# adelacvg/detail_tts

Measured on AMD Instinct MI355X. Metric: generated audio seconds/sec (24 kHz), 10 s prompt, batch 8 per GPU, higher is better.
Workload: dtype f32; 1 GPU; configs[2]: 1xMI355X batch-8, 10 s prompts (T_ref=936), 234 codes -> 9.984 s audio per utterance; GPT KV-cache decode + 50-step CFG diffusion + flow-VAE/HiFiGAN vocoder, seed-0 random-init weights; batch_per_gpu=8, codes=234, diffusion_steps=50, parallelism=replica x1

## Files before the change

detail_tts_amd/csrc/attention.h:

```cpp
#pragma once
#include "common.h"

namespace dtts {

struct AttnParams {
    const float* qkv = nullptr;
    long long bs = 0;
    int cs = 0;
    int q_off = 0, k_off = 0, v_off = 0, head_stride = 0;
    float* out = nullptr;
    long long o_bs = 0;
    int o_cs = 0;
    const int* lens = nullptr;
    int T = 0, B = 0, H = 0, D = 0;
    float scale = 1.f;
    const float* bias_tab = nullptr;
    int causal = 0;
    const float* band = nullptr;
    int band_w = 0;
    float* ml_out = nullptr;
    int layout_pad = 0;
    void* out_x3 = nullptr;
    int x3_tp = 0;
    const void* planes = nullptr;
    int p1 = 0;
    int ksplit = 1;
    int ksplit_max = 0;
    float* kpart = nullptr;
    int* kcount = nullptr;
};

struct AttnPlanes {
    static constexpr int D = 48, KT = 64, TILE_BYTES = 2 * (6 * 64 + 8 * 48) * 16;
    __host__ __device__ static inline int tq(int T) { return (T + KT - 1) / KT * KT; }
    __host__ __device__ static inline int nt64(int T) { return (T + KT - 1) / KT; }
    __host__ __device__ static inline size_t q_bytes(int T) { return (size_t)2 * 6 * tq(T) * 16; }
    __host__ __device__ static inline size_t head_bytes(int T) { return q_bytes(T) + (size_t)nt64(T) * TILE_BYTES; }
    __host__ __device__ static inline size_t bytes(int B, int H, int T) { return (size_t)B * H * head_bytes(T); }
};

struct AttnX3Launch {
    int ksplit = 0, p1 = 0, workgroups = 0;
};
void launch_flash_attention(const AttnParams& p, hipStream_t stream, AttnX3Launch* chosen = nullptr);
// ... 13 lines not shown
```

detail_tts_amd/csrc/attention_x3b.hip:

```cpp
#include <atomic>
#include <type_traits>

#include "attention.h"
#include "conv_x3.h"
#include "split3.h"

namespace dtts {

namespace {
typedef float f16v __attribute__((ext_vector_type(16)));

constexpr int D = 48, KT = 64, QPW = 32, BIAS_CLIP = 64;
constexpr int KCH = 6 * KT;
constexpr int NPL = XS_PLANES;
constexpr int KBYTES = NPL * KCH * 16;
constexpr int VPLANE_G = 8 * D * 16;
constexpr int VHALF = 4 * D * 16;
constexpr int VSLOT = NPL * VHALF;
constexpr int EXT_HALF = 128, EXT_N = 2 * EXT_HALF + 1;
constexpr int ONES_BYTES = VHALF + 2 * D * 16 + 16;
constexpr int LDS_K = 0, LDS_V = 2 * KBYTES, LDS_ONES = LDS_V + 4 * VSLOT, LDS_EXT = LDS_ONES + 16, LDS_BYTES = LDS_ONES + ONES_BYTES;
static_assert(16 + EXT_N * 4 <= 2 * D * 16, "the bias table fits between the two ones chunks");
static_assert(3 * ((LDS_BYTES + 511) / 512 * 512) <= 160 * 1024, "three workgroups per CU");
constexpr float QK_SCALE = 16.f, P_SHIFT = 10.f, V_SCALE = 16.f, M_SLACK = 3.f;
// ... 213 lines not shown
    asm volatile("s_nop 7\n\ts_nop 7\n\ts_nop 7" : "+v"(a), "+v"(b));
}

template <int MINB, bool KSPLIT = false, bool ONEP = false>
__global__ __launch_bounds__(256, MINB) void flash_attn_x3b_kernel(const AttnParams p) {
    constexpr float LOG2E = 1.4426950408889634f;
    constexpr int NW = 4, QPB = NW * QPW;
    extern __shared__ __attribute__((aligned(16))) unsigned char smem[];
    float* ext_s = reinterpret_cast<float*>(smem + LDS_EXT);

    const int tid = threadIdx.x, lane = tid & 63, wave = __builtin_amdgcn_readfirstlane(tid >> 6);
    const int q = lane & 31, hh = lane >> 5;
    const int nqb = (p.T + QPB - 1) / QPB;
    const int S = KSPLIT ? p.ksplit : 1;
    const int Lall = xcd_remap(blockIdx.x, gridDim.x);
    const int Lid = KSPLIT ? Lall / S : Lall, zsp = KSPLIT ? Lall - Lid * S : 0;
    const int qb = Lid % nqb, hb = Lid / nqb;
    const int b = hb % p.B, h = hb / p.B;
    const int len = p.lens ? p.lens[b] : p.T;
    const int q0 = qb * QPB;
    if (q0 >= len) return;
    const int Tq = AttnPlanes::tq(p.T);
    const unsigned char* himg = static_cast<const unsigned char*>(p.planes) + ((size_t)b * p.H + h) * AttnPlanes::head_bytes(p.T);
    const unsigned char* kvimg = himg + AttnPlanes::q_bytes(p.T);
    for (int i = tid; i < EXT_N; i += NW * 64) {
        int o = i - EXT_HALF;
        o = o < -BIAS_CLIP ? -BIAS_CLIP : (o > BIAS_CLIP ? BIAS_CLIP : o);
        ext_s[i] = p.bias_tab[h * (2 * BIAS_CLIP + 1) + o + BIAS_CLIP] * LOG2E;
    }
    if (tid < 16) {
        const int c = tid >> 2;
        reinterpret_cast<unsigned*>(smem + LDS_ONES + (c >> 1) * VHALF + (c & 1) * (2 * D * 16))[tid & 3] = (c >> 1) ? 0u : 0x4C004C00u;
    }
// ... 207 lines not shown

void launch_flash_attention_x3b(const AttnParams& p, hipStream_t stream, AttnX3Launch* chosen) {
    DTTS_REQUIRE(p.D == 48 && p.bias_tab && !p.causal && !p.band && !p.ml_out && p.planes, "attention_x3b covers head dim 48 with the T5 bias on operand images");
    constexpr int NW = 4;
    const int base = cdiv(p.T, NW * QPW) * p.H * p.B;
    const int ks_env = attn_ksplit();
    static const int ks_maxb = env_int("DTTS_ATTN_KSPLIT_MAXB", 2);
    const int ks_cus = attn_ksplit_cus();
    int S = 1;
    if (p.B <= ks_maxb && ks_env > 1) {
        S = ks_env;
        while (S > 1 && ((long long)base * S > ks_cus || AttnPlanes::nt64(p.T) < 2 * S || (size_t)base * S > X3_MAX_SLABS || (size_t)base * NW > X3_SPLIT_COUNTERS)) --S;
    }
    if (p.ksplit_max > 0) S = std::min(S, p.ksplit_max);
    AttnParams q = p;
    if (S > 1) {
        q.ksplit = S;
        x3_split_workspace(stream, (size_t)base * S, &q.kpart, &q.kcount);
    }
    if (chosen) {
        chosen->ksplit = S;
        chosen->p1 = p.p1 ? 1 : 0;
        chosen->workgroups = base * S;
    }
    auto go = [&](auto kern) {
        lds_optin(reinterpret_cast<const void*>(kern), LDS_BYTES);
        hipLaunchKernelGGL(kern, dim3(base * S), dim3(NW * 64), LDS_BYTES, stream, q);
    };
    if (S > 1) {
        if (p.p1) go(flash_attn_x3b_kernel<2, true, true>);
// ... 10 lines not shown
```

detail_tts_amd/csrc/conv_gemm.h:

```cpp
#pragma once
#include "common.h"

namespace dtts {

struct ConvParams {
    const float* x = nullptr;
    long long x_bs = 0;
    int x_cs = 0;
    const int* len_in = nullptr;
    const int* x_bidx = nullptr;
    int Tin = 0;
    const float* pro_ab = nullptr;
    int pro_act = ACT_NONE;
    float pro_slope = 0.f;
    const float* w = nullptr;
    const float* bias = nullptr;
    int Cin = 0, CinP = 0, Cout = 0, CoutP = 0, KW = 1, stride = 1, dil = 1, pad = 0;
    const float* badd = nullptr;
    int badd_bs = 0;
    int gate = GATE_NONE;
    int epi_act = ACT_NONE;
    float epi_slope = 0.f;
    float out_scale = 1.f;
    const float* res = nullptr;
// ... 18 lines not shown
    int qkv_heads = 0, qkv_nt64 = 0, qkv_tq = 0;
    float qkv_qscale = 1.f;
    const int* cols = nullptr;
    int ncols = 0, cols_b0 = 0;
    void* next3 = nullptr;
    int next_c8 = 0, next_tp = 0, next_halo = 0, next_act = ACT_NONE;
    float next_slope = 0.f;
    int* next_sat = nullptr;
    int ksplit = 1;
    int ksplit_max = 0;
    int p1 = 0;
    int epi_vec = 0;
    float* kpart = nullptr;
    int* kcount = nullptr;
    int ablate = 0;
};

void launch_conv_gemm(const ConvParams& p, hipStream_t stream);
void set_conv_small_tiles(int n);

}
```

detail_tts_amd/csrc/conv_x3.hip:

```cpp
#include <algorithm>
#include <atomic>
#include <cstdio>
#include <mutex>
#include <type_traits>
#include <utility>
#include <vector>

#include "conv_x3.h"
#include <cstdlib>
#include "prof.h"
#include "split3.h"

namespace dtts {

typedef float f32x16 __attribute__((ext_vector_type(16)));

namespace {
constexpr int NPL = XS_PLANES, NK = 2 * NPL;
constexpr int BM = 128, BN = X3_BN;
constexpr int WTILE = NK * BM * 16;
constexpr int XMAIN = NK * BN * 16;
constexpr int XBUF = XMAIN + NK * 2 * 16;

__global__ __launch_bounds__(256) void split_weights_kernel(const float* __restrict__ wp, int C8, int CoutP, uint4* __restrict__ out) {
// ... 3 lines not shown
#pragma unroll
    for (int e = 0; e < 8; ++e) v[e] = wp[((long long)tap * C8 * 8 + c8 * 8 + e) * CoutP + m] * XS_SCALE_W;
    uint4 q0, q1;
    split8(v, q0, q1);
    uint4* o = out + ((long long)(tap * C8 + c8) * NPL) * CoutP + m;
    o[0] = q0;
    o[CoutP] = q1;
}

template <int ACT, bool AB>
__global__ __launch_bounds__(256) void split_planes_kernel(const float* __restrict__ x, long long x_bs, int x_cs,
                                                          const float* __restrict__ ab, const int* __restrict__ lens, int T, int C8,
                                                          int Tp, uint4* __restrict__ out) {
    const int tp = blockIdx.x * 256 + threadIdx.x, c8 = blockIdx.y, b = blockIdx.z;
    if (tp >= Tp) return;
    const int t = tp - X3_HALO, len = lens ? lens[b] : T;
    uint4 q0 = make_uint4(0, 0, 0, 0), q1 = q0;
    if (t >= 0 && t < len) {
        const float* xr = x + (long long)b * x_bs + (long long)(c8 * 8) * x_cs + t;
        float v[8];
#pragma unroll
        for (int e = 0; e < 8; ++e) v[e] = xr[(long long)e * x_cs];
        if (AB) {
            const float* abr = ab + ((long long)b * C8 + c8) * 16;
#pragma unroll
            for (int e = 0; e < 8; ++e) v[e] = abr[2 * e] * v[e] + abr[2 * e + 1];
        }
        if (ACT == ACT_SILU) {
#pragma unroll
            for (int e = 0; e < 8; ++e) v[e] = v[e] * __frcp_rn(1.f + __expf(-v[e]));
        }
#pragma unroll
        for (int e = 0; e < 8; ++e) v[e] *= XS_SCALE_X;
        split8(v, q0, q1);
    }
    uint4* o = out + ((long long)(b * C8 + c8) * NPL) * Tp + tp;
    o[0] = q0;
    o[Tp] = q1;
}

template <int ACT>
__global__ __launch_bounds__(1024) void gn_split_planes_kernel(const float* __restrict__ x, long long x_bs, int x_cs,
                                                              const int* __restrict__ lens, int T, int C, int groups,
                                                              const float* __restrict__ gamma, const float* __restrict__ beta, float eps,
                                                              const float* __restrict__ ada, int ada_stride, int ada_bs, int Tp,
                                                              uint4* __restrict__ out, const int* __restrict__ ada_idx, int x_bmod) {
    __shared__ float red[2][16];
    __shared__ float sa[64], sd[64];
    const int g = blockIdx.x, b = blockIdx.y, tid = threadIdx.x, lane = tid & 63, wave = tid >> 6, nthr = blockDim.x;
// ... 79 lines not shown
                v[e] *= XS_SCALE_X;
            }
            split8(v, q0, q1);
        }
        uint4* o = out + ((long long)(b * C8 + g * c8n + c8l) * NPL) * Tp + tp;
        o[0] = q0;
        o[Tp] = q1;
    }
}

template <int ACT, int NI>
__global__ __launch_bounds__(1024) void gn_split_planes_reg_kernel(const float* __restrict__ x, long long x_bs, int x_cs,
                                                                  const int* __restrict__ lens, int T, int C, int groups,
                                                                  const float* __restrict__ gamma, const float* __restrict__ beta, float eps,
                                                                  const float* __restrict__ ada, int ada_stride, int ada_bs, int Tp,
                                                                  uint4* __restrict__ out, const int* __restrict__ ada_idx, int x_bmod) {
    __shared__ float red[2][16];
    __shared__ float sa[64], sd[64];
    const int g = blockIdx.x, b = blockIdx.y, tid = threadIdx.x, lane = tid & 63, wave = tid >> 6;
    const int len = lens ? lens[b] : T;
    const int cpg = C / groups, c8n = cpg >> 3, C8 = C >> 3, nitems = c8n * Tp;
    const float* xg = x + (long long)(x_bmod ? b % x_bmod : b) * x_bs + (long long)(g * cpg) * x_cs;
    const float k = xg[0];
    float v[NI][8];
    float s1 = 0.f, s2 = 0.f;
#pragma unroll
    for (int q = 0; q < NI; ++q) {
        const int item = tid + q * 1024, c8l = item / Tp, t = item - c8l * Tp - X3_HALO;
        const bool ok = item < nitems && t >= 0 && t < len;
        const float* xr = xg + (long long)(ok ? c8l * 8 : 0) * x_cs + (ok ? t : 0);
#pragma unroll
        for (int e = 0; e < 8; ++e) v[q][e] = xr[(long long)e * x_cs];
        if (ok) {
            float d[8];
#pragma unroll
            for (int e = 0; e < 8; ++e) d[e] = v[q][e] - k;
            s1 += ((d[0] + d[1]) + (d[2] + d[3])) + ((d[4] + d[5]) + (d[6] + d[7]));
            s2 += ((d[0] * d[0] + d[1] * d[1]) + (d[2] * d[2] + d[3] * d[3])) + ((d[4] * d[4] + d[5] * d[5]) + (d[6] * d[6] + d[7] * d[7]));
        }
    }
#pragma unroll
    for (int o = 32; o > 0; o >>= 1) {
        s1 += __shfl_xor(s1, o);
        s2 += __shfl_xor(s2, o);
    }
    if (lane == 0) { red[0][wave] = s1; red[1][wave] = s2; }
    __syncthreads();
    float S1 = 0.f, S2 = 0.f;
// ... 9 lines not shown
        float d = beta[c] - mean * a;
        if (ada) {
            const float* ad = ada + (ada_idx ? (long long)ada_idx[b] : (long long)b * ada_bs);
            const float sc = 1.f + ad[(long long)c * ada_stride], sh = ad[(long long)(C + c) * ada_stride];
            a *= sc;
            d = d * sc + sh;
        }
        sa[tid] = a;
        sd[tid] = d;
    }
    __syncthreads();
#pragma unroll
    for (int q = 0; q < NI; ++q) {
        const int item = tid + q * 1024;
        if (item >= nitems) continue;
        const int c8l = item / Tp, tp = item - c8l * Tp, t = tp - X3_HALO;
        uint4 q0 = make_uint4(0, 0, 0, 0), q1 = q0;
        if (t >= 0 && t < len) {
            float w[8];
#pragma unroll
            for (int e = 0; e < 8; ++e) {
                w[e] = sa[c8l * 8 + e] * v[q][e] + sd[c8l * 8 + e];
                if (ACT == ACT_SILU) w[e] = w[e] * __frcp_rn(1.f + __expf(-w[e]));
                w[e] *= XS_SCALE_X;
            }
            split8(w, q0, q1);
        }
        uint4* o = out + ((long long)(b * C8 + g * c8n + c8l) * NPL) * Tp + tp;
        o[0] = q0;
        o[Tp] = q1;
    }
}

template <int EPI, bool KW3, int NSTG, bool P1 = false>
__global__ __launch_bounds__(256, NSTG == 2 ? 3 : 2) void conv_x3_kernel(ConvParams p) {
    constexpr int KW = KW3 ? 3 : 1, D = NSTG - 1;
    constexpr int CB = P1 ? 4 : 2;
    constexpr int NT = P1 ? 2 : 3;
    auto chunk_of = [](int kind) { return P1 ? kind * NPL : (kind & 1) * NPL + (kind >> 1); };
    constexpr int XOFF = NSTG * WTILE;
    extern __shared__ __attribute__((aligned(16))) unsigned char smem[];
    const int tid = threadIdx.x, lane = tid & 63, wave = __builtin_amdgcn_readfirstlane(tid >> 6), l31 = lane & 31, lhi = lane >> 5;
    const int mtiles = p.CoutP / BM, ntiles = (p.Nout + BN - 1) / BN;
    const int Ls = xcd_remap(blockIdx.x, gridDim.x);
    const int S = p.ksplit, L = Ls / S, z = Ls - L * S;
    int mt = L % mtiles;
    int b = (L / mtiles) / ntiles;
    int nti = (L / mtiles) - b * ntiles;
    int bn = L / mtiles;
    if (EPI == 2 && mtiles > 6 && mtiles % 6 == 0 && !(p.ablate & 1024)) {
        const int nbn = p.cols ? p.ncols : ntiles * p.B, per_blk = 5 * mtiles, blk = L / per_blk, r = L - blk * per_blk;
        const int bn0 = blk * 5, nb = min(5, nbn - bn0), per_grp = nb * 6, mg = r / per_grp, r2 = r - mg * per_grp, bnl = r2 / 6;
        mt = mg * 6 + (r2 - bnl * 6);
        bn = bn0 + bnl;
        b = bn / ntiles;
        nti = bn - b * ntiles;
    }
    if (p.cols) {
        const int pk = __builtin_amdgcn_readfirstlane(p.cols[bn]);
        b = (pk >> 8) - p.cols_b0;
        nti = pk & 255;
    }
    const int m0 = mt * BM, n0 = nti * BN;
    const int nvalid = p.len_out ? p.len_out[b] : p.Nout;
    if (n0 >= nvalid) return;
    const int C8 = p.Cin >> 3, call = p.Cin >> (P1 ? 5 : 4), Tp = p.x3_tp;
    const int cbeg = (int)((long long)call * z / S), c16n = (int)((long long)call * (z + 1) / S) - cbeg, nks = KW * c16n;
    const int bin = p.x_bidx ? p.x_bidx[b] : b;
    const unsigned lane16 = (unsigned)lane * 16u;
    const unsigned char* wb8 = static_cast<const unsigned char*>(p.w3) + ((long long)m0 + (long long)(CB * cbeg) * NPL * p.CoutP) * 16;
    const unsigned char* xb8 = static_cast<const unsigned char*>(p.x3) +
                               ((long long)bin * C8 * NPL * Tp + n0 + (X3_HALO - p.pad) + (long long)(CB * cbeg) * NPL * Tp) * 16;
    const long long wtapB = (long long)C8 * NPL * p.CoutP * 16;
    const long long wblkB = (long long)CB * NPL * p.CoutP * 16;
    const long long xblkB = (long long)CB * NPL * Tp * 16;
    auto dma = [&](const unsigned char* g, int lds_off) {
        __builtin_amdgcn_global_load_lds((const __attribute__((address_space(1))) void*)(g + lane16),
                                         (__attribute__((address_space(3))) void*)(smem + lds_off), 16, 0, 0);
    };
    const int wkind = wave;
    const unsigned char* wq = wb8 + (long long)chunk_of(wkind) * p.CoutP * 16;
    const int wlds = wkind * (BM * 16);
    const unsigned char* xq = xb8 + (long long)chunk_of(wkind) * Tp * 16;
    const int xlds = XOFF + wkind * (BN * 16);
    long long x3o[3];
    int x3l[3];
#pragma unroll
    for (int t = 0; t < 3; ++t) {
        const int j = t * 4 + wave, kind = j / 3, cb = j - kind * 3;
        x3o[t] = ((long long)chunk_of(kind) * Tp + cb * 64) * 16;
        x3l[t] = XOFF + kind * (BN * 16) + cb * 1024;
    }
    const long long halo_lane = (lane < 2 * NK) ? (((long long)chunk_of(lane >> 1) * Tp + BN + (lane & 1)) * 16 - (long long)lane16) : 0;
    const unsigned char* xblk = xb8;
    auto issue_w = [&](int i, int stage) { dma(wq + i * 1024, stage * WTILE + wlds + i * 1024); };
    auto issue_x1 = [&](int i, int stage) { dma(xq + i * 1024, stage * XBUF + xlds + i * 1024); };
    auto issue_x3 = [&](int t, int stage) { dma(xblk + x3o[t], stage * XBUF + x3l[t]); };
    auto issue_halo = [&](int stage) {
        if (lane < 2 * NK)
            __builtin_amdgcn_global_load_lds((const __attribute__((address_space(1))) void*)(xblk + halo_lane + lane16),
                                             (__attribute__((address_space(3))) void*)(smem + XOFF + stage * XBUF + XMAIN), 16, 0, 0);
    };
    int itap = 0;
    auto next_w = [&]() {
        if (!KW3) wq += wblkB;
        else if (itap < 2) { wq += wtapB; ++itap; }
        else { wq += wblkB - 2 * wtapB; itap = 0; }
    };

    const int wm0 = (wave >> 1) * 64, wn0 = (wave & 1) * 96;
    f32x16 acc[2][3];
#pragma unroll
    for (int i = 0; i < 2; ++i)
#pragma unroll
        for (int j = 0; j < 3; ++j)
#pragma unroll
            for (int r = 0; r < 16; ++r) acc[i][j][r] = 0.f;

#pragma unroll
    for (int q = 0; q < D; ++q) {
        if (q < nks) {
            issue_w(0, q);
            issue_w(1, q);
        }
        next_w();
        if (!KW3) {
            if (q < nks) {
#pragma unroll
                for (int i = 0; i < 3; ++i) issue_x1(i, q);
            }
            xq += xblkB;
        } else {
            if (q < c16n) {
#pragma unroll
                for (int t = 0; t < 3; ++t) issue_x3(t, q);
                issue_halo(q);
            }
            xblk += xblkB;
        }
    }
    float* bias_s = reinterpret_cast<float*>(smem + XOFF + NSTG * XBUF);
    if (tid < BM) bias_s[tid] = (p.bias && m0 + tid < p.Cout) ? p.bias[m0 + tid] : 0.f;

    int c16 = 0, tap = 0;
    int sw = 0, sx = 0;
    auto read_frags = [&](hf8 (&fa)[2][NPL], hf8 (&fb)[3][NPL], int stw, int stx, int tp) {
        const unsigned char* As = smem + stw * WTILE + lhi * (BM * 16);
        const unsigned char* Xb = smem + XOFF + stx * XBUF;
#pragma unroll
        for (int j = 0; j < 3; ++j) {
            const int nn = wn0 + j * 32 + l31 + tp;
            const unsigned char* xr = nn < BN ? Xb + lhi * (BN * 16) + nn * 16 : Xb + XMAIN + lhi * 32 + (nn - BN) * 16;
            const int xps = nn < BN ? 2 * BN * 16 : 64;
#pragma unroll
            for (int pl = 0; pl < NPL; ++pl) fb[j][pl] = *reinterpret_cast<const hf8*>(xr + pl * xps);
        }
#pragma unroll
// ... 74 lines not shown
#pragma unroll
        for (; slot < 5; ++slot) uslot(slot);
        if (!KW3) {
            wq += wblkB;
            xq += xblkB;
        } else {
            if ((TAPc + D) % KW < 2) wq += wtapB;
            else wq += wblkB - 2 * wtapB;
            if (TAPc == KW - 1) xblk += xblkB;
        }
    };
    auto uperiod = [&](auto... kc) { (ustep(kc), ...); };
    constexpr bool UNROLL = KW3 || EPI == 2;
    if (UNROLL && !(p.ablate & 512)) {
        const int nper = KW3 ? (c16n - D) / NSTG : (nks - D) / PERIOD;
        for (int q = 0; q < nper; ++q) {
            if constexpr (PERIOD == 2) uperiod(std::integral_constant<int, 0>{}, std::integral_constant<int, 1>{});
            else if constexpr (PERIOD == 3) uperiod(std::integral_constant<int, 0>{}, std::integral_constant<int, 1>{}, std::integral_constant<int, 2>{});
            else if constexpr (PERIOD == 4) uperiod(std::integral_constant<int, 0>{}, std::integral_constant<int, 1>{}, std::integral_constant<int, 2>{}, std::integral_constant<int, 3>{});
            else if constexpr (PERIOD == 6) uperiod(std::integral_constant<int, 0>{}, std::integral_constant<int, 1>{}, std::integral_constant<int, 2>{}, std::integral_constant<int, 3>{}, std::integral_constant<int, 4>{}, std::integral_constant<int, 5>{});
            else if constexpr (PERIOD == 9) uperiod(std::integral_constant<int, 0>{}, std::integral_constant<int, 1>{}, std::integral_constant<int, 2>{}, std::integral_constant<int, 3>{}, std::integral_constant<int, 4>{}, std::integral_constant<int, 5>{}, std::integral_constant<int, 6>{}, std::integral_constant<int, 7>{}, std::integral_constant<int, 8>{});
            else uperiod(std::integral_constant<int, 0>{}, std::integral_constant<int, 1>{}, std::integral_constant<int, 2>{}, std::integral_constant<int, 3>{}, std::integral_constant<int, 4>{}, std::integral_constant<int, 5>{}, std::integral_constant<int, 6>{}, std::integral_constant<int, 7>{}, std::integral_constant<int, 8>{}, std::integral_constant<int, 9>{}, std::integral_constant<int, 10>{}, std::integral_constant<int, 11>{});
        }
        ks = nper * PERIOD;
        c16 = ks / KW;
        itap = D % KW;
    }
    for (; ks < nks; ++ks) {
        if (NSTG == 2 || ks + D > nks || (KW3 && c16 + D >= c16n)) asm volatile("s_waitcnt vmcnt(0)" ::: "memory");
        else asm volatile("s_waitcnt vmcnt(%0)" ::"n"((NSTG - 2) * (KW3 ? 3 : 5)) : "memory");
        __builtin_amdgcn_s_barrier();
        read_frags(a, bb, sw, sx, tap);
        const int swi = sw + D >= NSTG ? sw + D - NSTG : sw + D, sxi = sx + D >= NSTG ? sx + D - NSTG : sx + D;
        const bool wlive = ks + D < nks, xlive = KW3 ? c16 + D < c16n : ks + D < nks;
        int slot = 0;
#pragma unroll
        for (int t = 0; t < NT; ++t)
#pragma unroll
            for (int i = 0; i < 2; ++i) {
#pragma unroll
                for (int j = 0; j < 3; ++j) acc[i][j] = __builtin_amdgcn_mfma_f32_32x32x16_f16(a[i][TA[t]], bb[j][TB[t]], acc[i][j], 0, 0, 0);
                if (slot < 5) issue_slot(slot, swi, sxi, wlive, xlive);
                ++slot;
            }
// ... 322 lines not shown
}

void launch_gn_split_planes(const float* x, long long x_bs, int x_cs, const int* lens, int T, int B, int C, int groups,
                            const float* gamma, const float* beta, float eps, const float* ada, int ada_stride, int ada_bs, int act,
                            void* out, hipStream_t s, const int* ada_idx, int x_bmod) {
    DTTS_REQUIRE(C % groups == 0 && (C / groups) % 8 == 0 && C / groups <= 64, "gn_split_planes: group size");
    DTTS_REQUIRE(act == ACT_NONE || act == ACT_SILU, "gn_split_planes: activation");
    const int Tp = x3_tp(T);
    uint4* o = static_cast<uint4*>(out);
    ProfScope ps("gn_split_planes_kernel", 0.0, (double)B * C * T * 8.0, s);
    static const int ns = env_int("DTTS_GN_SPLIT_NS", 1);
    static const int nt = env_int("DTTS_GN_SPLIT_NT", 1024);
    static const bool reg_ok = env_on("DTTS_GN_SPLIT_REG");
    constexpr int NI = 3;
    if (reg_ok && ns == 1 && (C / groups / 8) * Tp <= NI * 1024) {
        if (act == ACT_SILU)
            hipLaunchKernelGGL((gn_split_planes_reg_kernel<ACT_SILU, NI>), dim3(groups, B), dim3(1024), 0, s, x, x_bs, x_cs, lens, T, C, groups,
                               gamma, beta, eps, ada, ada_stride, ada_bs, Tp, o, ada_idx, x_bmod);
        else
            hipLaunchKernelGGL((gn_split_planes_reg_kernel<ACT_NONE, NI>), dim3(groups, B), dim3(1024), 0, s, x, x_bs, x_cs, lens, T, C, groups,
                               gamma, beta, eps, ada, ada_stride, ada_bs, Tp, o, ada_idx, x_bmod);
        DTTS_CHECK_HIP(hipGetLastError());
        return;
    }
    if (act == ACT_SILU)
        hipLaunchKernelGGL(gn_split_planes_kernel<ACT_SILU>, dim3(groups, B, ns), dim3(nt), 0, s, x, x_bs, x_cs, lens, T, C, groups, gamma,
                           beta, eps, ada, ada_stride, ada_bs, Tp, o, ada_idx, x_bmod);
    else
        hipLaunchKernelGGL(gn_split_planes_kernel<ACT_NONE>, dim3(groups, B, ns), dim3(nt), 0, s, x, x_bs, x_cs, lens, T, C, groups, gamma,
                           beta, eps, ada, ada_stride, ada_bs, Tp, o, ada_idx, x_bmod);
    DTTS_CHECK_HIP(hipGetLastError());
}

namespace {
struct KSplitWs {
    float* part;
// ... 85 lines not shown
    const long long ntile_pad = (long long)(p.CoutP / BM) * cdiv(p.Nout, BN) * p.B;
    static const int max_split_k1 = env_int("DTTS_CONV_KSPLIT_K1", 2);
    if (ntile_pad <= split_tiles) S = (int)std::min<long long>(std::min<long long>(p.KW == 3 ? max_split : std::min(max_split, max_split_k1), split_wgs / ntile_pad), (p.Cin >> 4) / 8);
    if (p.ksplit_max > 0) S = std::min(S, p.ksplit_max);
    if (S < 1) S = 1;
    p.ksplit = S;
    static const bool epi_vec_on = env_on("DTTS_X3_EPI_VEC");
    auto al16 = [](const void* q, long long bs, int cs) { return (reinterpret_cast<unsigned long long>(q) & 15ull) == 0 && (bs & 3) == 0 && (cs & 3) == 0; };
    p.epi_vec = (epi_vec_on && p.y && al16(p.y, p.y_bs, p.y_cs) && (!p.res || al16(p.res, p.res_bs, p.res_cs))) ? 1 : 0;
    if (S > 1) {
        const KSplitWs w = ksplit_workspace(s, (size_t)ntile * S);
        p.kpart = w.part;
        p.kcount = w.count;
    }
    const long long nwg = ntile * S;
    static const long long max4k3 = env_int("DTTS_CONV_STAGES4_MAXWG_K3", 128);
    const int nstg = force_stg ? force_stg : (nwg <= (p.KW == 3 ? max4k3 : max4) ? 4 : (nwg <= max3 ? 3 : 2));
    const size_t lds = (size_t)nstg * (WTILE + XBUF) + BM * sizeof(float) + 16;
    const int l4 = 4 * (WTILE + XBUF) + BM * (int)sizeof(float) + 16;
    const dim3 grid((unsigned)nwg);
    const double cols = (double)p.B * p.Nout;
    const double flops = 2.0 * p.Cout * p.Cin * p.KW * cols;
    const double bytes = 4.0 * cols * p.Cin + 4.0 * cols * p.Cout * (p.res ? 2.0 : 1.0) + 4.0 * (double)p.Cout * p.Cin * p.KW;
    {
        static const bool by_shape = []() { const char* v = env_str("DTTS_PROF_SHAPES"); return v && v[0] == '1'; }();
        const char* tag = p1 ? "conv_x3_kernel<128,192,fp16>" : "conv_x3_kernel<128,192>";
        if (by_shape && p1) tag = p.KW == 3 ? "conv_x3 fp16 k3" : (p.Cout > 1024 ? "conv_x3 fp16 k1 M=2304" : (p.res ? "conv_x3 fp16 k1 +res" : "conv_x3 fp16 k1"));
        else if (by_shape) tag = p.KW == 3 ? "conv_x3 k3" : (p.Cout > 1024 ? "conv_x3 k1 M=2304" : (p.res ? "conv_x3 k1 +res" : "conv_x3 k1"));
        ProfScope ps(tag, flops, bytes, s);
        const bool epi = p.epi_act != ACT_NONE || p.out_scale != 1.f;
// ... 49 lines not shown
```

detail_tts_amd/csrc/model.h:

```cpp
#pragma once
#include <map>
#include <memory>
#include <atomic>
#include <thread>
#include <cstring>
#include <memory>
#include <mutex>
#include <string>
#include <unordered_map>
#include <vector>

#include "attention.h"
#include "attn_probs.h"
#include "common.h"
#include "conv_gemm.h"
#include "conv_x3.h"
#include "diff_loss.h"
#include "diff_schedule.h"
#include "disc.h"
#include "flowvae_fwd.h"
#include "gpt_kernels.h"
#include "ops.h"
#include "../../include/detail_hip.h"

// ... 414 lines not shown
    hipGraphExec_t gpt_capture(int n);
    void gpt_drop_graphs();
    void build_vq();
    void build_frontend();
    void gpt_prefill_layers(float* x, const int* lens, int B, int L, float* kv_cache, long long kv_layer_stride, long long kv_bs,
                            int kv_cs, hipStream_t s, const GptAttnCapture* capture = nullptr);
    void gpt_capture_probs(const GptAttnCapture& c, int layer, const float* qkv, const int* lens, int B, int L, hipStream_t s);
    MelStyleW mel_style_w(const std::string& prefix, int n_mel, int hidden, int out) const;
    ConvParams cp(const float* x, int cin, float* y, int cout, int B, int T, int Ta, const int* lens) const;
    ConvParams cp(const float* x, int cin, int Tin, int Tin_a, const int* len_in, float* y, int cout, int Nout, int Nout_a, const int* len_out,
                  int B) const;
    static void with_planes(ConvParams& p, const void* xs, int T) { p.x3 = xs; p.x3_tp = x3_tp(T); }
    static void with_res(ConvParams& p, const float* res, long long bs, int cs) { p.res = res; p.res_bs = bs; p.res_cs = cs; }

    const int* upload_ints(const int* host, int n, hipStream_t s);
    void register_cols(const int* lens_dev, const int* lens_host, int nb, int T, hipStream_t s);

    void run_conv(const PackedConv& pc, ConvParams p, hipStream_t s, ConvX3Launch* chosen = nullptr) const;
    struct TrunkIo {
        const int* lens;
        int B, T, Ta;
        hipStream_t s;
        float* ab;
        void* xs = nullptr;
        bool p1 = false;
        const int* step_idx = nullptr;
    };
    void norm_input(const float* x, int C, const float* gamma, const float* beta, int act, bool x3, const TrunkIo& io);
    void attention_block(const AttnBlockW& w, const float* x, float* y, float* qkv, float* att, const TrunkIo& io);
    void res_block_fwd(const Schedule& sc, const ResBlockW& w, const float* x, float* h1, float* y, int step, const TrunkIo& io);
// ... 178 lines not shown
```

detail_tts_amd/csrc/model.hip:

```cpp
#include "model.h"
#include <algorithm>
#include <cmath>
#include <cstring>

namespace dtts {

static thread_local Arena* t_arena_override = nullptr;
Arena* arena_override() { return t_arena_override; }
ArenaUse::ArenaUse(Arena& a) : prev_(t_arena_override) { t_arena_override = &a; }
ArenaUse::~ArenaUse() { t_arena_override = prev_; }

static thread_local bool t_row_invariant = false;
RowInvariantLaunches::RowInvariantLaunches() : prev_(t_row_invariant) { t_row_invariant = true; }
RowInvariantLaunches::~RowInvariantLaunches() { t_row_invariant = prev_; }
bool RowInvariantLaunches::on() { return t_row_invariant; }

Arena::~Arena() {
    if (base_) (void)hipFree(base_);
}

void Arena::ensure(size_t bytes) {
    if (bytes > cap_) {
        DTTS_CHECK_HIP(hipDeviceSynchronize());
        if (base_) DTTS_CHECK_HIP(hipFree(base_));
// ... 113 lines not shown
    for (int g = first; g <= last; ++g)
        if (std::find(r.users[g].begin(), r.users[g].end(), s) == r.users[g].end()) r.users[g].push_back(s);
    int* dst = r.dev + r.off;
    int* stage = r.pinned + r.off;
    r.off += len;
    for (size_t i = t_col_tables.size(); i-- > 0;) {
        const ColTable& e = t_col_tables[i];
        auto hit = [&](const int* q, int m) { return q < dst + len && dst < q + m; };
        if (hit(e.lens, e.nb) || hit(e.cols, e.prefix.back())) t_col_tables.erase(t_col_tables.begin() + (long)i);
    }
    if (n > 0) {
        std::memcpy(stage, host, sizeof(int) * (size_t)n);
        DTTS_CHECK_HIP(hipMemcpyAsync(dst, stage, sizeof(int) * (size_t)n, hipMemcpyHostToDevice, s));
    }
    return dst;
}

void Model::register_cols(const int* lens_dev, const int* lens_host, int nb, int T, hipStream_t s) {
    for (size_t i = t_col_tables.size(); i-- > 0;)
        if (t_col_tables[i].lens == lens_dev) t_col_tables.erase(t_col_tables.begin() + (long)i);
    if (!col_tables_on() || !opt_conv_cols_ || !lens_dev || !lens_host || nb <= 0 || cdiv(T, X3_BN) >= 256) return;
    const int nt = cdiv(T, X3_BN);
    ColTable e;
    e.prefix.assign(1, 0);
    std::vector<int> tab;
    for (int b = 0; b < nb; ++b) {
        const int live = std::min(nt, cdiv(std::max(lens_host[b], 0), X3_BN));
        for (int i = 0; i < live; ++i) tab.push_back(b << 8 | i);
        e.prefix.push_back((int)tab.size());
    }
// ... 389 lines not shown
```

detail_tts_amd/csrc/model_diffusion.hip:

```cpp
#include "model.h"
#include <algorithm>
#include <cmath>
#include <cstring>
#include "prof.h"

namespace dtts {

static void make_masked_stream(hipStream_t* st, int cus) {
    uint32_t mask[8] = {0, 0, 0, 0, 0, 0, 0, 0};
    for (int b = 0; b < cus; ++b) mask[b >> 5] |= 1u << (b & 31);
    DTTS_CHECK_HIP(hipExtStreamCreateWithCUMask(st, 8, mask));
}

static void make_side_stream(hipStream_t* st) {
    static const int reserve = env_int("DTTS_B_CU_RESERVE", 0);
    if (reserve > 0 && reserve < 256) make_masked_stream(st, 256 - reserve);
    else DTTS_CHECK_HIP(hipStreamCreateWithFlags(st, hipStreamNonBlocking));
}

void Model::ensure_fork_events() {
    if (ev_fork_) return;
    DTTS_CHECK_HIP(hipEventCreateWithFlags(&ev_fork_, hipEventDisableTiming));
    for (auto& e : ev_joinx_) DTTS_CHECK_HIP(hipEventCreateWithFlags(&e, hipEventDisableTiming));
}
// ... 331 lines not shown
        const int len = lens_host ? lens_host[b] : T;
        l2[b] = l2[B + b] = len;
        li.push_back(len);
        um[b] = b;
        um[2 * B + b] = um[3 * B + b] = b;
        int gidx = -1;
        for (size_t k = 0; k < ul.size(); ++k)
            if (ul[k] == len) gidx = (int)k;
        if (gidx < 0) { gidx = (int)ul.size(); ul.push_back(len); }
        um[B + b] = B + gidx;
    }
    for (int v : ul) li.push_back(v);
    PairPlan pl;
    pl.Nu = (int)ul.size();
    pl.ulen = ul;
    pl.lens2 = upload_ints(l2.data(), 2 * B, s);
    pl.lens_i = upload_ints(li.data(), (int)li.size(), s);
    pl.umap = upload_ints(um.data(), 4 * B, s);
    pl.xmap = pl.umap + 2 * B;
    register_cols(pl.lens2, l2.data(), 2 * B, T, s);
    register_cols(pl.lens_i, li.data(), (int)li.size(), T, s);
    return pl;
}

void Model::diff_forward_pair(const Schedule& sc, const float* x, const float* cbuf0, const PairPlan& pl, int B, int T, int step, float* out2,
                              hipStream_t s, const float* integ) {
    const int C = cfg.diff_channels, Ta = T, OC = cfg.diff_out_channels, MC = cfg.mel_channels, Nu = pl.Nu;
    const int *lens2 = pl.lens2, *lens_i = pl.lens_i;
    const long long bs = (long long)C * Ta;
    static const bool env_two = env_on("DTTS_TWO_STREAMS");
    const bool two_streams = env_two && opt_two_streams_;
    const bool x3 = use_x3();
// ... 29 lines not shown
            res_block_fwd(sc, integ_[l].rb, in, tA, tB, step, io);
            attention_block(integ_[l].at, tB, bufI, qkv, tA, io);
            in = bufI;
        }
        code_half(bufI, bufP, io);
        ws().rewind(mark);
        P = bufP;
    }
    if (NS > 1) {
        DTTS_CHECK_HIP(hipEventRecord(ev_fork_, s));
        for (int k = 1; k < NS; ++k) DTTS_CHECK_HIP(hipStreamWaitEvent(sx_[k - 1], ev_fork_, 0));
    }
    for (int k = 0; k < NS; ++k) {
        hipStream_t st = k ? sx_[k - 1] : s;
        const int b0 = k * n;
        const int* lens = lens2 + b0;
        const size_t act = (size_t)n * C * Ta;
        float* bufA = ws().f32(act);
        float* bufB = ws().f32(act);
        float* bufC = ws().f32(act);
        float* qkv = ws().f32(qkv_floats(n, C, T));
        TrunkIo io{lens, n, T, Ta, st, ws().f32((size_t)n * C * 2)};
        io.xs = x3 ? ws().raw(x3_bytes(n, C, T)) : nullptr;
        ConvParams r = cp(x, MC, T, T, lens, bufB, C, T, Ta, lens, n);
        r.pad = 1;
        r.x_bidx = pl.xmap + b0;
        with_res(r, P, bs, Ta);
        r.res_bidx = pl.umap + b0;
        if (x3) with_planes(r, xs0, T);
        run_conv(xpath_, r, st);
        float* cur = bufB;
// ... 149 lines not shown
        DTTS_CHECK_HIP(hipStreamWaitEvent(side, ev_fork_, 0));
    }
    std::vector<int> lv(Bv), sv(Bv), bv(Bv);
    int ci = 0;
    const int prof_rot = prof_rot_++;
    for (int k0 = 0; k0 < NS; k0 += J, ++ci) {
        const Lane& L = lanes[two ? (ci & 1) : 0];
        Profiler::gate() = ((ci / 2 + prof_rot) % Profiler::get().step_every) == 0;
        const int jn = std::min(J, NS - k0), nb = jn * Bi;
        for (int j = 0; j < jn; ++j)
            for (int b = 0; b < Bi; ++b) {
                lv[j * Bi + b] = lens_i_host[b];
                sv[j * Bi + b] = steps[k0 + j];
                bv[j * Bi + b] = b;
            }
        const int* dl = upload_ints(lv.data(), nb, L.st);
        const int* ds = upload_ints(sv.data(), nb, L.st);
        const int* db = x3 ? nullptr : upload_ints(bv.data(), nb, L.st);
        register_cols(dl, lv.data(), nb, T, L.st);
        float* outp = integ_all + (size_t)k0 * Bi * ct;
        TrunkIo io{dl, nb, T, T, L.st, L.ab};
        io.xs = L.xs;
        io.step_idx = ds;
        auto dlayer = [&](const DiffLayerW& l, const float* in, float* o) {
            res_block_fwd(sc, l.rb, in, L.bufB, L.bufC, 0, io);
            attention_block(l.at, L.bufC, o, L.qkv, L.bufB, io);
        };
        res_block_back(sc, integ_[0].rb, h1, cbuf0, L.bufC, 0, io, Bi, db);
        attention_block(integ_[0].at, L.bufC, L.bufA, L.qkv, L.bufB, io);
        dlayer(integ_[1], L.bufA, L.bufA);
        dlayer(integ_[2], L.bufA, L.bufA);
// ... 411 lines not shown
        attention_block(blk, cur, nxt, qkv, att, io);
        std::swap(cur, nxt);
    }
    launch_gn_coeffs(cur, bs, nmax, dl, nmax, B, C, gn_groups(C), code_gn_g_, code_gn_b_, 1e-5f, cond, 1, 2 * C, io.ab, s);
    launch_affine_apply(cur, bs, nmax, io.ab, dl, nmax, B, C, 4, ACT_NONE, code_emb, (long long)C * 4 * nmax, 4 * nmax, s);
}

void Model::op_attention_block(const char* prefix, const float* x, const int* lens_host, int B, int C, int T, float* y,
                               hipStream_t s) {
    DTTS_REQUIRE(bound_, "weights not bound");
    AttnBlockW w = attn_block(prefix, C, cfg.diff_heads);
    const size_t act = (size_t)B * C * T;
    ws().ensure(sizeof(float) * (act + qkv_floats(B, C, T) + (size_t)2 * B * C) + x3_bytes(B, C, T) + 8192);
    std::vector<int> l(B);
    for (int b = 0; b < B; ++b) l[b] = lens_host ? lens_host[b] : T;
    const int* dl = upload_ints(l.data(), B, s);
    float* qkv = ws().f32(qkv_floats(B, C, T));
    float* att = ws().f32(act);
    TrunkIo io{dl, B, T, T, s, ws().f32((size_t)2 * B * C)};
    for (auto* grp : {&integ_, &layers_})
        for (size_t i = 0; i < grp->size(); ++i)
            if ((*grp)[i].at.qkv.w == w.qkv.w) {
                w = (*grp)[i].at;
                io.p1 = opt_trunk_fp16_ && grp == &layers_ && i >= 1;
            }
    io.xs = (use_x3() && w.qkv.w3) ? ws().raw(x3_bytes(B, C, T)) : nullptr;
    attention_block(w, x, y, qkv, att, io);
}

void Model::op_resblock(const char* prefix, const float* x, const int* lens_host, int B, int T, int step, float* y,
                        hipStream_t s) {
// ... 2 lines not shown
    const int C = cfg.diff_channels;
    const ResBlockW* found = nullptr;
    const std::string pf(prefix);
    bool p1 = false;
    auto check = [&](const ResBlockW& r, const std::string& name, bool covered) {
        if (name == pf) { found = &r; p1 = opt_trunk_fp16_ && covered; }
    };
    for (size_t i = 0; i < integ_.size(); ++i) check(integ_[i].rb, "diffusion.conditioning_timestep_integrator." + std::to_string(i) + ".resblk", false);
    for (size_t i = 0; i < layers_.size(); ++i) check(layers_[i].rb, "diffusion.layers." + std::to_string(i) + ".resblk", i >= 1);
    for (size_t i = 0; i < tail_.size(); ++i) check(tail_[i], "diffusion.layers." + std::to_string(layers_.size() + i), true);
    DTTS_REQUIRE(found, "unknown resblock prefix");
    const size_t act = (size_t)B * C * T;
    ws().ensure(sizeof(float) * (act + (size_t)2 * B * C) + x3_bytes(B, C, T) + 8192);
    std::vector<int> l(B);
    for (int b = 0; b < B; ++b) l[b] = lens_host ? lens_host[b] : T;
    const int* dl = upload_ints(l.data(), B, s);
    float* h1 = ws().f32(act);
    TrunkIo io{dl, B, T, T, s, ws().f32((size_t)2 * B * C)};
    io.xs = use_x3() ? ws().raw(x3_bytes(B, C, T)) : nullptr;
    io.p1 = p1;
    res_block_fwd(sched0_, *found, x, h1, y, step, io);
}

}
```

Baseline: 185.2 audio_s/s.

## Use precomputed fast division for tile decode, defer conv x loads, skip full-length lens

Adds a FastDiv multiply-shift helper and uses host-precomputed divisors for workgroup index decoding in the attention and conv_x3 kernels and in the group-norm split kernel. The conv_x3 kernel now issues weight prefetches before resolving the column/batch and the early-exit check, then adds finer-grained vmcnt waits for the first stages. Split-plane kernels load unconditionally and mask afterwards. Lens arrays that all equal T are replaced by nullptr, which skips the upload and the per-kernel length loads. Risks include fastdiv correctness for near-limit dividends, the fixed vmcnt counts being wrong, and (n0 + Nout) behaviour changes when lens are null.

```diff
diff --git a/detail_tts_amd/csrc/attention.h b/detail_tts_amd/csrc/attention.h
--- a/detail_tts_amd/csrc/attention.h
+++ b/detail_tts_amd/csrc/attention.h
@@ -1,5 +1,6 @@
 #pragma once
 #include "common.h"
+#include "tile_decode.h"
 
 namespace dtts {
 
@@ -28,6 +29,7 @@
     int ksplit_max = 0;
     float* kpart = nullptr;
     int* kcount = nullptr;
+    FastDiv td_ksplit, td_nqb, td_B;
 };
 
 struct AttnPlanes {
diff --git a/detail_tts_amd/csrc/attention_x3b.hip b/detail_tts_amd/csrc/attention_x3b.hip
--- a/detail_tts_amd/csrc/attention_x3b.hip
+++ b/detail_tts_amd/csrc/attention_x3b.hip
@@ -251,9 +251,9 @@
     const int nqb = (p.T + QPB - 1) / QPB;
     const int S = KSPLIT ? p.ksplit : 1;
     const int Lall = xcd_remap(blockIdx.x, gridDim.x);
-    const int Lid = KSPLIT ? Lall / S : Lall, zsp = KSPLIT ? Lall - Lid * S : 0;
-    const int qb = Lid % nqb, hb = Lid / nqb;
-    const int b = hb % p.B, h = hb / p.B;
+    const int Lid = KSPLIT ? (int)fastdiv((unsigned)Lall, p.td_ksplit) : Lall, zsp = KSPLIT ? Lall - Lid * S : 0;
+    const int hb = (int)fastdiv((unsigned)Lid, p.td_nqb), qb = Lid - hb * nqb;
+    const int h = (int)fastdiv((unsigned)hb, p.td_B), b = hb - h * p.B;
     const int len = p.lens ? p.lens[b] : p.T;
     const int q0 = qb * QPB;
     if (q0 >= len) return;
@@ -491,6 +491,9 @@
     }
     if (p.ksplit_max > 0) S = std::min(S, p.ksplit_max);
     AttnParams q = p;
+    DTTS_REQUIRE((long long)base * S <= (long long)FASTDIV_MAX_DIVIDEND && fastdiv_make((uint32_t)S, &q.td_ksplit) &&
+                     fastdiv_make((uint32_t)cdiv(p.T, NW * QPW), &q.td_nqb) && fastdiv_make((uint32_t)p.B, &q.td_B),
+                 "attention_x3b: launch size");
     if (S > 1) {
         q.ksplit = S;
         x3_split_workspace(stream, (size_t)base * S, &q.kpart, &q.kcount);
diff --git a/detail_tts_amd/csrc/conv_gemm.h b/detail_tts_amd/csrc/conv_gemm.h
--- a/detail_tts_amd/csrc/conv_gemm.h
+++ b/detail_tts_amd/csrc/conv_gemm.h
@@ -1,5 +1,6 @@
 #pragma once
 #include "common.h"
+#include "tile_decode.h"
 
 namespace dtts {
 
@@ -56,6 +57,8 @@
     float* kpart = nullptr;
     int* kcount = nullptr;
     int ablate = 0;
+    int td_mtiles = 0, td_ntiles = 0, td_tall = 0;
+    FastDiv td_ksplit, td_m, td_n, td_blk, td_grp, td_grp_tail;
 };
 
 void launch_conv_gemm(const ConvParams& p, hipStream_t stream);
diff --git a/detail_tts_amd/csrc/conv_x3.hip b/detail_tts_amd/csrc/conv_x3.hip
--- a/detail_tts_amd/csrc/conv_x3.hip
+++ b/detail_tts_amd/csrc/conv_x3.hip
@@ -41,9 +41,9 @@
                                                           int Tp, uint4* __restrict__ out) {
     const int tp = blockIdx.x * 256 + threadIdx.x, c8 = blockIdx.y, b = blockIdx.z;
     if (tp >= Tp) return;
-    const int t = tp - X3_HALO, len = lens ? lens[b] : T;
+    const int t = tp - X3_HALO;
     uint4 q0 = make_uint4(0, 0, 0, 0), q1 = q0;
-    if (t >= 0 && t < len) {
+    if (t >= 0 && t < T) {
         const float* xr = x + (long long)b * x_bs + (long long)(c8 * 8) * x_cs + t;
         float v[8];
 #pragma unroll
@@ -60,6 +60,7 @@
 #pragma unroll
         for (int e = 0; e < 8; ++e) v[e] *= XS_SCALE_X;
         split8(v, q0, q1);
+        if (t >= (lens ? lens[b] : T)) q0 = q1 = make_uint4(0, 0, 0, 0);
     }
     uint4* o = out + ((long long)(b * C8 + c8) * NPL) * Tp + tp;
     o[0] = q0;
@@ -169,24 +170,30 @@
                                                                   const int* __restrict__ lens, int T, int C, int groups,
                                                                   const float* __restrict__ gamma, const float* __restrict__ beta, float eps,
                                                                   const float* __restrict__ ada, int ada_stride, int ada_bs, int Tp,
-                                                                  uint4* __restrict__ out, const int* __restrict__ ada_idx, int x_bmod) {
+                                                                  uint4* __restrict__ out, const int* __restrict__ ada_idx, int x_bmod,
+                                                                  int cpg, FastDiv rTp) {
     __shared__ float red[2][16];
     __shared__ float sa[64], sd[64];
     const int g = blockIdx.x, b = blockIdx.y, tid = threadIdx.x, lane = tid & 63, wave = tid >> 6;
-    const int len = lens ? lens[b] : T;
-    const int cpg = C / groups, c8n = cpg >> 3, C8 = C >> 3, nitems = c8n * Tp;
+    const int c8n = cpg >> 3, C8 = C >> 3, nitems = c8n * Tp;
     const float* xg = x + (long long)(x_bmod ? b % x_bmod : b) * x_bs + (long long)(g * cpg) * x_cs;
     const float k = xg[0];
     float v[NI][8];
+    int tq[NI];
+#pragma unroll
+    for (int q = 0; q < NI; ++q) {
+        const int item = tid + q * 1024, c8l = (int)fastdiv((unsigned)item, rTp), t = item - c8l * Tp - X3_HALO;
+        const bool in = item < nitems && t >= 0 && t < T;
+        tq[q] = in ? t : T;
+        const float* xr = xg + (long long)(in ? c8l * 8 : 0) * x_cs + (in ? t : 0);
+#pragma unroll
+        for (int e = 0; e < 8; ++e) v[q][e] = xr[(long long)e * x_cs];
+    }
+    const int len = lens ? lens[b] : T;
     float s1 = 0.f, s2 = 0.f;
 #pragma unroll
     for (int q = 0; q < NI; ++q) {
-        const int item = tid + q * 1024, c8l = item / Tp, t = item - c8l * Tp - X3_HALO;
-        const bool ok = item < nitems && t >= 0 && t < len;
-        const float* xr = xg + (long long)(ok ? c8l * 8 : 0) * x_cs + (ok ? t : 0);
-#pragma unroll
-        for (int e = 0; e < 8; ++e) v[q][e] = xr[(long long)e * x_cs];
-        if (ok) {
+        if (tq[q] < len) {
             float d[8];
 #pragma unroll
             for (int e = 0; e < 8; ++e) d[e] = v[q][e] - k;
@@ -226,7 +233,7 @@
     for (int q = 0; q < NI; ++q) {
         const int item = tid + q * 1024;
         if (item >= nitems) continue;
-        const int c8l = item / Tp, tp = item - c8l * Tp, t = tp - X3_HALO;
+        const int c8l = (int)fastdiv((unsigned)item, rTp), tp = item - c8l * Tp, t = tp - X3_HALO;
         uint4 q0 = make_uint4(0, 0, 0, 0), q1 = q0;
         if (t >= 0 && t < len) {
             float w[8];
@@ -253,36 +260,23 @@
     constexpr int XOFF = NSTG * WTILE;
     extern __shared__ __attribute__((aligned(16))) unsigned char smem[];
     const int tid = threadIdx.x, lane = tid & 63, wave = __builtin_amdgcn_readfirstlane(tid >> 6), l31 = lane & 31, lhi = lane >> 5;
-    const int mtiles = p.CoutP / BM, ntiles = (p.Nout + BN - 1) / BN;
-    const int Ls = xcd_remap(blockIdx.x, gridDim.x);
-    const int S = p.ksplit, L = Ls / S, z = Ls - L * S;
-    int mt = L % mtiles;
-    int b = (L / mtiles) / ntiles;
-    int nti = (L / mtiles) - b * ntiles;
-    int bn = L / mtiles;
-    if (EPI == 2 && mtiles > 6 && mtiles % 6 == 0 && !(p.ablate & 1024)) {
-        const int nbn = p.cols ? p.ncols : ntiles * p.B, per_blk = 5 * mtiles, blk = L / per_blk, r = L - blk * per_blk;
-        const int bn0 = blk * 5, nb = min(5, nbn - bn0), per_grp = nb * 6, mg = r / per_grp, r2 = r - mg * per_grp, bnl = r2 / 6;
+    const int mtiles = p.td_mtiles, ntiles = p.td_ntiles;
+    const unsigned Ls = (unsigned)xcd_remap(blockIdx.x, gridDim.x);
+    const int S = p.ksplit, L = (int)fastdiv(Ls, p.td_ksplit), z = (int)Ls - L * S;
+    int bn = (int)fastdiv((unsigned)L, p.td_m);
+    int mt = L - bn * mtiles;
+    if (EPI == 2 && p.td_tall) {
+        const int nbn = p.cols ? p.ncols : ntiles * p.B, per_blk = 5 * mtiles, blk = (int)fastdiv((unsigned)L, p.td_blk), r = L - blk * per_blk;
+        const int bn0 = blk * 5, nb = min(5, nbn - bn0), per_grp = nb * 6;
+        const int mg = (int)fastdiv((unsigned)r, nb == 5 ? p.td_grp : p.td_grp_tail), r2 = r - mg * per_grp, bnl = r2 / 6;
         mt = mg * 6 + (r2 - bnl * 6);
         bn = bn0 + bnl;
-        b = bn / ntiles;
-        nti = bn - b * ntiles;
-    }
-    if (p.cols) {
-        const int pk = __builtin_amdgcn_readfirstlane(p.cols[bn]);
-        b = (pk >> 8) - p.cols_b0;
-        nti = pk & 255;
-    }
-    const int m0 = mt * BM, n0 = nti * BN;
-    const int nvalid = p.len_out ? p.len_out[b] : p.Nout;
-    if (n0 >= nvalid) return;
+    }
+    const int m0 = mt * BM;
     const int C8 = p.Cin >> 3, call = p.Cin >> (P1 ? 5 : 4), Tp = p.x3_tp;
-    const int cbeg = (int)((long long)call * z / S), c16n = (int)((long long)call * (z + 1) / S) - cbeg, nks = KW * c16n;
-    const int bin = p.x_bidx ? p.x_bidx[b] : b;
+    const int cbeg = (int)fastdiv((unsigned)(call * z), p.td_ksplit), c16n = (int)fastdiv((unsigned)(call * (z + 1)), p.td_ksplit) - cbeg, nks = KW * c16n;
     const unsigned lane16 = (unsigned)lane * 16u;
     const unsigned char* wb8 = static_cast<const unsigned char*>(p.w3) + ((long long)m0 + (long long)(CB * cbeg) * NPL * p.CoutP) * 16;
-    const unsigned char* xb8 = static_cast<const unsigned char*>(p.x3) +
-                               ((long long)bin * C8 * NPL * Tp + n0 + (X3_HALO - p.pad) + (long long)(CB * cbeg) * NPL * Tp) * 16;
     const long long wtapB = (long long)C8 * NPL * p.CoutP * 16;
     const long long wblkB = (long long)CB * NPL * p.CoutP * 16;
     const long long xblkB = (long long)CB * NPL * Tp * 16;
@@ -293,7 +287,7 @@
     const int wkind = wave;
     const unsigned char* wq = wb8 + (long long)chunk_of(wkind) * p.CoutP * 16;
     const int wlds = wkind * (BM * 16);
-    const unsigned char* xq = xb8 + (long long)chunk_of(wkind) * Tp * 16;
+    const unsigned char* xq = nullptr;
     const int xlds = XOFF + wkind * (BN * 16);
     long long x3o[3];
     int x3l[3];
@@ -304,7 +298,7 @@
         x3l[t] = XOFF + kind * (BN * 16) + cb * 1024;
     }
     const long long halo_lane = (lane < 2 * NK) ? (((long long)chunk_of(lane >> 1) * Tp + BN + (lane & 1)) * 16 - (long long)lane16) : 0;
-    const unsigned char* xblk = xb8;
+    const unsigned char* xblk = nullptr;
     auto issue_w = [&](int i, int stage) { dma(wq + i * 1024, stage * WTILE + wlds + i * 1024); };
     auto issue_x1 = [&](int i, int stage) { dma(xq + i * 1024, stage * XBUF + xlds + i * 1024); };
     auto issue_x3 = [&](int t, int stage) { dma(xblk + x3o[t], stage * XBUF + x3l[t]); };
@@ -321,14 +315,21 @@
     };
 
     const int wm0 = (wave >> 1) * 64, wn0 = (wave & 1) * 96;
-    f32x16 acc[2][3];
-#pragma unroll
-    for (int i = 0; i < 2; ++i)
-#pragma unroll
-        for (int j = 0; j < 3; ++j)
-#pragma unroll
-            for (int r = 0; r < 16; ++r) acc[i][j][r] = 0.f;
-
+
+    float bias_v = 0.f;
+    if (tid < BM && p.bias && m0 + tid < p.Cout) bias_v = p.bias[m0 + tid];
+    int b, nti;
+    if (p.cols) {
+        const int pk = __builtin_amdgcn_readfirstlane(p.cols[bn]);
+        b = (pk >> 8) - p.cols_b0;
+        nti = pk & 255;
+    } else {
+        b = (int)fastdiv((unsigned)bn, p.td_n);
+        nti = bn - b * ntiles;
+    }
+    const int n0 = nti * BN;
+    const int nvalid = p.len_out ? p.len_out[b] : p.Nout;
+    const int bin = p.x_bidx ? p.x_bidx[b] : b;
 #pragma unroll
     for (int q = 0; q < D; ++q) {
         if (q < nks) {
@@ -336,6 +337,17 @@
             issue_w(1, q);
         }
         next_w();
+    }
+    if (n0 >= nvalid) {
+        asm volatile("s_waitcnt vmcnt(0)" ::: "memory");
+        return;
+    }
+    const unsigned char* xb8 = static_cast<const unsigned char*>(p.x3) +
+                               ((long long)bin * C8 * NPL * Tp + n0 + (X3_HALO - p.pad) + (long long)(CB * cbeg) * NPL * Tp) * 16;
+    xq = xb8 + (long long)chunk_of(wkind) * Tp * 16;
+    xblk = xb8;
+#pragma unroll
+    for (int q = 0; q < D; ++q) {
         if (!KW3) {
             if (q < nks) {
 #pragma unroll
@@ -351,8 +363,15 @@
             xblk += xblkB;
         }
     }
+    f32x16 acc[2][3];
+#pragma unroll
+    for (int i = 0; i < 2; ++i)
+#pragma unroll
+        for (int j = 0; j < 3; ++j)
+#pragma unroll
+            for (int r = 0; r < 16; ++r) acc[i][j][r] = 0.f;
     float* bias_s = reinterpret_cast<float*>(smem + XOFF + NSTG * XBUF);
-    if (tid < BM) bias_s[tid] = (p.bias && m0 + tid < p.Cout) ? p.bias[m0 + tid] : 0.f;
+    if (tid < BM) bias_s[tid] = bias_v;
 
     int c16 = 0, tap = 0;
     int sw = 0, sx = 0;
@@ -457,6 +476,7 @@
     constexpr bool UNROLL = KW3 || EPI == 2;
     if (UNROLL && !(p.ablate & 512)) {
         const int nper = KW3 ? (c16n - D) / NSTG : (nks - D) / PERIOD;
+        if (!KW3 && NSTG >= 3 && nper > 0) asm volatile("s_waitcnt vmcnt(3)" ::: "memory");
         for (int q = 0; q < nper; ++q) {
             if constexpr (PERIOD == 2) uperiod(std::integral_constant<int, 0>{}, std::integral_constant<int, 1>{});
             else if constexpr (PERIOD == 3) uperiod(std::integral_constant<int, 0>{}, std::integral_constant<int, 1>{}, std::integral_constant<int, 2>{});
@@ -471,6 +491,8 @@
     }
     for (; ks < nks; ++ks) {
         if (NSTG == 2 || ks + D > nks || (KW3 && c16 + D >= c16n)) asm volatile("s_waitcnt vmcnt(0)" ::: "memory");
+        else if (!KW3 && ks == 0) asm volatile("s_waitcnt vmcnt(%0)" ::"n"(3 * (D - 1)) : "memory");
+        else if (!KW3 && D > 2 && ks == 1) asm volatile("s_waitcnt vmcnt(%0)" ::"n"(D > 2 ? 3 * (D - 2) + 5 : 0) : "memory");
         else asm volatile("s_waitcnt vmcnt(%0)" ::"n"((NSTG - 2) * (KW3 ? 3 : 5)) : "memory");
         __builtin_amdgcn_s_barrier();
         read_frags(a, bb, sw, sx, tap);
@@ -823,12 +845,15 @@
     static const bool reg_ok = env_on("DTTS_GN_SPLIT_REG");
     constexpr int NI = 3;
     if (reg_ok && ns == 1 && (C / groups / 8) * Tp <= NI * 1024) {
+        FastDiv rTp;
+        DTTS_REQUIRE(fastdiv_make((uint32_t)Tp, &rTp), "gn_split_planes: time padding");
+        const int cpg = C / groups;
         if (act == ACT_SILU)
             hipLaunchKernelGGL((gn_split_planes_reg_kernel<ACT_SILU, NI>), dim3(groups, B), dim3(1024), 0, s, x, x_bs, x_cs, lens, T, C, groups,
-                               gamma, beta, eps, ada, ada_stride, ada_bs, Tp, o, ada_idx, x_bmod);
+                               gamma, beta, eps, ada, ada_stride, ada_bs, Tp, o, ada_idx, x_bmod, cpg, rTp);
         else
             hipLaunchKernelGGL((gn_split_planes_reg_kernel<ACT_NONE, NI>), dim3(groups, B), dim3(1024), 0, s, x, x_bs, x_cs, lens, T, C, groups,
-                               gamma, beta, eps, ada, ada_stride, ada_bs, Tp, o, ada_idx, x_bmod);
+                               gamma, beta, eps, ada, ada_stride, ada_bs, Tp, o, ada_idx, x_bmod, cpg, rTp);
         DTTS_CHECK_HIP(hipGetLastError());
         return;
     }
@@ -944,6 +969,18 @@
         p.kcount = w.count;
     }
     const long long nwg = ntile * S;
+    {
+        const int mtiles = p.CoutP / BM, ntiles = cdiv(p.Nout, BN);
+        const long long nbn = p.cols ? p.ncols : (long long)ntiles * p.B;
+        DTTS_REQUIRE(nwg <= (long long)FASTDIV_MAX_DIVIDEND && (long long)(p.Cin >> 4) * S <= (long long)FASTDIV_MAX_DIVIDEND, "conv_x3: launch too large");
+        p.td_mtiles = mtiles;
+        p.td_ntiles = ntiles;
+        p.td_tall = (mtiles > 6 && mtiles % 6 == 0 && !(p.ablate & 1024)) ? 1 : 0;
+        const bool ok = fastdiv_make((uint32_t)S, &p.td_ksplit) && fastdiv_make((uint32_t)mtiles, &p.td_m) && fastdiv_make((uint32_t)ntiles, &p.td_n) &&
+                        fastdiv_make((uint32_t)(5 * mtiles), &p.td_blk) && fastdiv_make(30u, &p.td_grp) &&
+                        fastdiv_make((uint32_t)(6 * std::max<long long>(1, nbn % 5)), &p.td_grp_tail);
+        DTTS_REQUIRE(ok, "conv_x3: tile counts");
+    }
     static const long long max4k3 = env_int("DTTS_CONV_STAGES4_MAXWG_K3", 128);
     const int nstg = force_stg ? force_stg : (nwg <= (p.KW == 3 ? max4k3 : max4) ? 4 : (nwg <= max3 ? 3 : 2));
     const size_t lds = (size_t)nstg * (WTILE + XBUF) + BM * sizeof(float) + 16;
diff --git a/detail_tts_amd/csrc/model.h b/detail_tts_amd/csrc/model.h
--- a/detail_tts_amd/csrc/model.h
+++ b/detail_tts_amd/csrc/model.h
@@ -452,6 +452,7 @@
     static void with_res(ConvParams& p, const float* res, long long bs, int cs) { p.res = res; p.res_bs = bs; p.res_cs = cs; }
 
     const int* upload_ints(const int* host, int n, hipStream_t s);
+    const int* upload_lens(const int* host, int n, int T, hipStream_t s);
     void register_cols(const int* lens_dev, const int* lens_host, int nb, int T, hipStream_t s);
 
     void run_conv(const PackedConv& pc, ConvParams p, hipStream_t s, ConvX3Launch* chosen = nullptr) const;
diff --git a/detail_tts_amd/csrc/model.hip b/detail_tts_amd/csrc/model.hip
--- a/detail_tts_amd/csrc/model.hip
+++ b/detail_tts_amd/csrc/model.hip
@@ -151,6 +151,12 @@
         DTTS_CHECK_HIP(hipMemcpyAsync(dst, stage, sizeof(int) * (size_t)n, hipMemcpyHostToDevice, s));
     }
     return dst;
+}
+
+const int* Model::upload_lens(const int* host, int n, int T, hipStream_t s) {
+    bool full = true;
+    for (int i = 0; i < n; ++i) full = full && host[i] == T;
+    return full ? nullptr : upload_ints(host, n, s);
 }
 
 void Model::register_cols(const int* lens_dev, const int* lens_host, int nb, int T, hipStream_t s) {
diff --git a/detail_tts_amd/csrc/model_diffusion.hip b/detail_tts_amd/csrc/model_diffusion.hip
--- a/detail_tts_amd/csrc/model_diffusion.hip
+++ b/detail_tts_amd/csrc/model_diffusion.hip
@@ -369,8 +369,8 @@
     PairPlan pl;
     pl.Nu = (int)ul.size();
     pl.ulen = ul;
-    pl.lens2 = upload_ints(l2.data(), 2 * B, s);
-    pl.lens_i = upload_ints(li.data(), (int)li.size(), s);
+    pl.lens2 = upload_lens(l2.data(), 2 * B, T, s);
+    pl.lens_i = upload_lens(li.data(), (int)li.size(), T, s);
     pl.umap = upload_ints(um.data(), 4 * B, s);
     pl.xmap = pl.umap + 2 * B;
     register_cols(pl.lens2, l2.data(), 2 * B, T, s);
@@ -430,7 +430,7 @@
     for (int k = 0; k < NS; ++k) {
         hipStream_t st = k ? sx_[k - 1] : s;
         const int b0 = k * n;
-        const int* lens = lens2 + b0;
+        const int* lens = lens2 ? lens2 + b0 : nullptr;
         const size_t act = (size_t)n * C * Ta;
         float* bufA = ws().f32(act);
         float* bufB = ws().f32(act);
@@ -610,7 +610,7 @@
                 sv[j * Bi + b] = steps[k0 + j];
                 bv[j * Bi + b] = b;
             }
-        const int* dl = upload_ints(lv.data(), nb, L.st);
+        const int* dl = upload_lens(lv.data(), nb, T, L.st);
         const int* ds = upload_ints(sv.data(), nb, L.st);
         const int* db = x3 ? nullptr : upload_ints(bv.data(), nb, L.st);
         register_cols(dl, lv.data(), nb, T, L.st);
@@ -1052,7 +1052,7 @@
     ws().ensure(sizeof(float) * (act + qkv_floats(B, C, T) + (size_t)2 * B * C) + x3_bytes(B, C, T) + 8192);
     std::vector<int> l(B);
     for (int b = 0; b < B; ++b) l[b] = lens_host ? lens_host[b] : T;
-    const int* dl = upload_ints(l.data(), B, s);
+    const int* dl = upload_lens(l.data(), B, T, s);
     float* qkv = ws().f32(qkv_floats(B, C, T));
     float* att = ws().f32(act);
     TrunkIo io{dl, B, T, T, s, ws().f32((size_t)2 * B * C)};
@@ -1085,7 +1085,7 @@
     ws().ensure(sizeof(float) * (act + (size_t)2 * B * C) + x3_bytes(B, C, T) + 8192);
     std::vector<int> l(B);
     for (int b = 0; b < B; ++b) l[b] = lens_host ? lens_host[b] : T;
-    const int* dl = upload_ints(l.data(), B, s);
+    const int* dl = upload_lens(l.data(), B, T, s);
     float* h1 = ws().f32(act);
     TrunkIo io{dl, B, T, T, s, ws().f32((size_t)2 * B * C)};
     io.xs = use_x3() ? ws().raw(x3_bytes(B, C, T)) : nullptr;
diff --git a/detail_tts_amd/csrc/tile_decode.h b/detail_tts_amd/csrc/tile_decode.h
--- /dev/null
+++ b/detail_tts_amd/csrc/tile_decode.h
@@ -0,0 +1,44 @@
+#pragma once
+#include <cstdint>
+
+#if defined(__HIPCC__) || defined(__CUDACC__)
+#define TILE_DECODE_HD __host__ __device__
+#else
+#define TILE_DECODE_HD
+#endif
+
+namespace dtts {
+
+struct FastDiv {
+    uint32_t mul = 0, shift = 0;
+};
+
+constexpr uint32_t FASTDIV_MAX_DIVIDEND = 0x7fffffffu;
+
+inline bool fastdiv_make(uint32_t d, FastDiv* out) {
+    if (d < 1 || d > 0x80000000u) return false;
+    uint32_t s = 0;
+    while ((uint64_t(1) << s) < d) ++s;
+    const uint64_t pw = uint64_t(1) << (32 + s);
+    const uint64_t m = pw / d + (pw % d ? 1 : 0);
+    out->mul = (uint32_t)(m - (uint64_t(1) << 32));
+    out->shift = s;
+    return true;
+}
+
+TILE_DECODE_HD inline uint32_t fastdiv_mulhi(uint32_t a, uint32_t b) {
+#if defined(__HIP_DEVICE_COMPILE__)
+    return __umulhi(a, b);
+#else
+    return (uint32_t)(((uint64_t)a * b) >> 32);
+#endif
+}
+
+TILE_DECODE_HD inline uint32_t fastdiv(uint32_t n, FastDiv f) { return (fastdiv_mulhi(n, f.mul) + n) >> f.shift; }
+
+TILE_DECODE_HD inline void fastdivmod(uint32_t n, FastDiv f, uint32_t d, uint32_t* q, uint32_t* r) {
+    *q = fastdiv(n, f);
+    *r = n - *q * d;
+}
+
+}
```

Result: no change. 186.5 audio_s/s, median of 6 (+0.7%).
